# bmezaris/RetargetVid

Hardware: AMD Instinct MI355X
Metric: frames/sec end-to-end saliency+crop on 640x360 (higher is better)
Workload: dtype f32

## Files before the change

### retargetvid_amd/csrc/svc_net.hip

```cpp
#include <math.h>

#include <algorithm>

#include "svc_internal.h"
#include "svc_x3.h"

static inline int ceil_div(int a, int b) { return (a + b - 1) / b; }

__device__ __forceinline__ unsigned xcd_bx() {
    const unsigned b = blockIdx.x, n = gridDim.x;
    return (n & 7) ? b : (b & 7) * (n >> 3) + (b >> 3);
}

typedef float f32x2 __attribute__((ext_vector_type(2)));
__device__ __forceinline__ void fma4(float4 &a, const float4 x, const float4 w) {
    const f32x2 lo = __builtin_elementwise_fma((f32x2){x.x, x.y}, (f32x2){w.x, w.y}, (f32x2){a.x, a.y});
    const f32x2 hi = __builtin_elementwise_fma((f32x2){x.z, x.w}, (f32x2){w.z, w.w}, (f32x2){a.z, a.w});
    a = make_float4(lo.x, lo.y, hi.x, hi.y);
}


static thread_local char g_err[512] = "";
void svc_set_error(const char *fmt, ...) {
    va_list ap;
// ... 713 lines not shown
        }
#pragma unroll
        for (int ty = 0; ty < TY; ++ty) {
            const int ky = r - ty;
            if (ky < 0 || ky > 2) continue;
#pragma unroll
            for (int tx = 0; tx < TX; ++tx)
#pragma unroll
                for (int kx = 0; kx < 3; ++kx) {
                    const float4 x = row[tx + kx], ww = w[ky * 3 + kx];
                    acc[ty][tx].x = fmaf(x.x, ww.x, acc[ty][tx].x);
                    acc[ty][tx].y = fmaf(x.y, ww.y, acc[ty][tx].y);
                    acc[ty][tx].z = fmaf(x.z, ww.z, acc[ty][tx].z);
                    acc[ty][tx].w = fmaf(x.w, ww.w, acc[ty][tx].w);
                }
        }
    }
    const float4 b = *(const float4 *)(bias + c4 * 4);
    float *yf = Y + (size_t)f * H * W * C + c4 * 4;
#pragma unroll
    for (int ty = 0; ty < TY; ++ty)
#pragma unroll
        for (int tx = 0; tx < TX; ++tx) {
            if (oy0 + ty >= H || ox0 + tx >= W) continue;
            float4 v = acc[ty][tx];
            v.x = fminf(fmaxf(v.x + b.x, 0.f), 6.f);
            v.y = fminf(fmaxf(v.y + b.y, 0.f), 6.f);
            v.z = fminf(fmaxf(v.z + b.z, 0.f), 6.f);
            v.w = fminf(fmaxf(v.w + b.w, 0.f), 6.f);
            *(float4 *)(yf + ((size_t)(oy0 + ty) * W + ox0 + tx) * C) = v;
        }
}

__global__ __launch_bounds__(256) void k_subsample(const float *__restrict__ X, float *__restrict__ Y, int n, int H,
                                                   int W, int C) {
    const int C4 = C >> 2, OH = H >> 1, OW = W >> 1;
    size_t gid = (size_t)blockIdx.x * 256 + threadIdx.x;
    size_t total = (size_t)n * OH * OW * C4;
    if (gid >= total) return;
    int c4 = gid % C4;
    size_t pix = gid / C4;
    int ox = pix % OW, oy = (pix / OW) % OH, f = pix / ((size_t)OW * OH);
    *(float4 *)(Y + gid * 4) = *(const float4 *)(X + (((size_t)f * H + 2 * oy) * W + 2 * ox) * C + c4 * 4);
}

__global__ __launch_bounds__(256) void k_gauss_fill(const float *__restrict__ G, float *__restrict__ Y, int n,
                                                    int npos, int ldy, int c_off) {
    size_t gid = (size_t)blockIdx.x * 256 + threadIdx.x;
    size_t total = (size_t)n * npos * 16;
    if (gid >= total) return;
    int j = gid & 15;
    size_t fp = gid >> 4;
    int pos = fp % npos;
    Y[fp * ldy + c_off + j] = G[pos * 16 + j];
}

__global__ __launch_bounds__(256) void k_adapt(const float *__restrict__ X, const float *__restrict__ w,
                                               const float *__restrict__ b, float *__restrict__ Y, size_t npix,
                                               unsigned *__restrict__ fmax, int n, unsigned long long *__restrict__ census, int ncen) {
    size_t gid = (size_t)blockIdx.x * 256 + threadIdx.x;
    if (gid < (size_t)n) fmax[gid] = 0;
    if (census && gid < (size_t)ncen) {
        unsigned *pf = (unsigned *)(census + 4) + gid * 4;
#pragma unroll
        for (int j = 0; j < 3; ++j)
            if (pf[j]) { atomicAdd(census + j, (unsigned long long)pf[j]); pf[j] = 0; }
    }
    if (gid >= npix) return;
    const float4 *x = (const float4 *)(X + gid * 64);
    const float4 *w4 = (const float4 *)w;
    float s = 0.f;
#pragma unroll
    for (int i = 0; i < 16; ++i) {
        float4 a = x[i], c = w4[i];
        s = fmaf(a.x, c.x, s);
        s = fmaf(a.y, c.y, s);
        s = fmaf(a.z, c.z, s);
        s = fmaf(a.w, c.w, s);
    }
    Y[gid] = s + b[0];
}

__device__ __forceinline__ unsigned enc_f32(float v) {
    unsigned u = __float_as_uint(v);
    return (u & 0x80000000u) ? ~u : (u | 0x80000000u);
}
__device__ __forceinline__ float dec_f32(unsigned u) {
    return __uint_as_float((u & 0x80000000u) ? (u & 0x7FFFFFFFu) : ~u);
}

#ifdef SD_PACKED
#define SD_NO_PK
#else
#define SD_NO_PK SVC_NO_PK
#endif
__device__ __forceinline__ float sd_bilinear(float lx0, float lx1, float ly0, float ly1, float a00, float a01, float a10, float a11) {
#ifdef SD_PACKED
    return ly0 * (lx0 * a00 + lx1 * a01) + ly1 * (lx0 * a10 + lx1 * a11);
#else
    float p00, p01, p10, p11, r0, r1, q0, q1, v;
    asm volatile("v_mul_f32 %0, %1, %2" : "=v"(p00) : "v"(lx0), "v"(a00));
    asm volatile("v_mul_f32 %0, %1, %2" : "=v"(p01) : "v"(lx1), "v"(a01));
    asm volatile("v_mul_f32 %0, %1, %2" : "=v"(p10) : "v"(lx0), "v"(a10));
    asm volatile("v_mul_f32 %0, %1, %2" : "=v"(p11) : "v"(lx1), "v"(a11));
    asm volatile("v_add_f32 %0, %1, %2" : "=v"(r0) : "v"(p00), "v"(p01));
    asm volatile("v_add_f32 %0, %1, %2" : "=v"(r1) : "v"(p10), "v"(p11));
    asm volatile("v_mul_f32 %0, %1, %2" : "=v"(q0) : "v"(ly0), "v"(r0));
    asm volatile("v_mul_f32 %0, %1, %2" : "=v"(q1) : "v"(ly1), "v"(r1));
    asm volatile("v_add_f32 %0, %1, %2" : "=v"(v) : "v"(q0), "v"(q1));
    return v;
#endif
}

// ... 496 lines not shown
        SVC_CHECK_LAUNCH();
        return SVC_OK;
    }
    svc_set_error("no pointwise kernel for K = %d, N = %d%s", K, N, R ? " with a residual" : ups ? " with an up-sampled term" : "");
    return SVC_E_INVALID;
}

static int launch_pw(SvcHandle *h, hipStream_t s, const float *X, int ldx, const SvcLayer &L, const float *R, int ldr,
                     float *Y, int ldy, int M, int n) {
    return launch_pw_ex(h, s, X, ldx, L.w.dev, L.cin, L.cin, L.b.dev, L.relu6, L.cout, R, ldr, Y, ldy, M, n, nullptr);
}

static int launch_dw(SvcHandle *h, hipStream_t s, const float *X, const SvcLayer &L, float *Y, int n, int H, int W) {
    ProfScope ps(h, SVC_K_DW, s);
    const int C = L.cout, GX = (W + 3) / 4, GY = (H + 1) / 2;
    const size_t cells = (size_t)n * GY * GX * (C / 4);
    k_dw_tile<4, 2><<<blocks256(cells), 256, 0, s>>>(X, L.w.dev, L.b.dev, Y, n, H, W, C, make_fdiv(C / 4), make_fdiv(GX),
                                                     make_fdiv(GY), (uint32_t)cells);
    SVC_CHECK_LAUNCH();
    return SVC_OK;
}

#define IRB_ES 36
#ifndef IRB_XREG
#define IRB_XREG 1
#endif
#ifndef IRB_WAVES
#define IRB_WAVES 4
#endif
#ifndef IRB_STAMP
#define IRB_STAMP(i)
#endif

template <int NT, int PW, int NWV, bool MX = false>
__global__ __launch_bounds__(64 * NWV) __attribute__((amdgpu_waves_per_eu(2, 8))) void k_dwpw(const float *__restrict__ X, int H, int W, int C,
                                              const float *__restrict__ Wd, const float *__restrict__ bd,
                                              const float *__restrict__ Wp, const float *__restrict__ bp, int N,
                                              int Npad, const float *__restrict__ R, int ldr, float *__restrict__ Y,
                                              int ldy, int relu6, int tiles_x, int tiles_y, int lw_tiles) {
    constexpr int PH = 32 / PW;
    __shared__ float smem_dwpw[NWV * 32 * IRB_ES + NWV * 16 * 64];
    float (*Dw)[32 * IRB_ES] = (float (*)[32 * IRB_ES])smem_dwpw;
    float (*red)[16][64] = (float (*)[16][64])(smem_dwpw + NWV * 32 * IRB_ES);
    const int tid = threadIdx.x, lane = tid & 63, wave = tid >> 6, r = lane & 31, hh = lane >> 5;
    int bid = xcd_bx();
    const int tx = bid % tiles_x;
    bid /= tiles_x;
    const int ty = bid % tiles_y, f = bid / tiles_y;
    const int x0 = tx * PW, y0 = ty * PH, n0 = blockIdx.y * (NT * 32);
    const int c4 = lane & 7, p0 = (lane >> 3) * 4;
    const int py = p0 / PW, pxs = p0 % PW;
    const int oy = y0 + py, ox0 = x0 + pxs;
    const float *xf = X + (size_t)f * H * W * C;
    float *D = Dw[wave];
    f32x16 acc[NT];
#pragma unroll
    for (int t = 0; t < NT; ++t)
#pragma unroll
        for (int i = 0; i < 16; ++i) acc[t][i] = 0.f;
    const int nchunks = (C + 31) >> 5;
    constexpr bool PRE = false;
    const float *wrow[NT];
#pragma unroll
    for (int t = 0; t < NT; ++t)
        wrow[t] = lw_tiles ? Wp + ((size_t)min((int)blockIdx.y * NT + t, lw_tiles - 1) * 64 + lane) * 4
                           : Wp + (size_t)min(n0 + t * 32 + r, Npad - 1) * C + 4 * hh;
    const size_t wstep = lw_tiles ? (size_t)lw_tiles * 256 : 8;
    for (int ch = wave; ch < nchunks; ch += NWV) {
        const int kend = min(32, C - ch * 32);
        float4 Bw[PRE ? NT : 1][4];
        if (PRE) {
#pragma unroll
            for (int t = 0; t < NT; ++t)
#pragma unroll
                for (int q = 0; q < 4; ++q)
                    Bw[PRE ? t : 0][q] = *(const float4 *)(wrow[t] + wstep * (ch * 4 + min(q, (kend >> 3) - 1)));
        }
        const int c = ch * 32 + c4 * 4;
        const bool cok = c < C;
        const int cc = cok ? c : 0;
        float4 o[4];
#pragma unroll
        for (int j = 0; j < 4; ++j) o[j] = make_float4(0.f, 0.f, 0.f, 0.f);
        {
            float4 w[9];
#pragma unroll
            for (int t = 0; t < 9; ++t) w[t] = *(const float4 *)(Wd + (size_t)t * C + cc);
// ... 102 lines not shown
            }
        }
        __builtin_amdgcn_wave_barrier();
    }
    const int yy = y0 + r / PW, xx = x0 + r % PW;
    const bool live = yy < H && xx < W;
    const size_t pix = ((size_t)f * H + yy) * W + xx;
#pragma unroll
    for (int t = 0; t < NT; ++t) {
        if (t) __syncthreads();
#pragma unroll
        for (int i = 0; i < 16; ++i) red[wave][i][lane] = acc[t][i];
        __syncthreads();
        if (wave >= 4) continue;
        const int g = wave;
        const int col = n0 + t * 32 + 8 * g + 4 * hh;
        if (col >= N || !live) continue;
        float4 v = make_float4(red[0][4 * g][lane], red[0][4 * g + 1][lane], red[0][4 * g + 2][lane], red[0][4 * g + 3][lane]);
#pragma unroll
        for (int q = 1; q < NWV; ++q) {
            v.x += red[q][4 * g][lane]; v.y += red[q][4 * g + 1][lane];
            v.z += red[q][4 * g + 2][lane]; v.w += red[q][4 * g + 3][lane];
        }
        const float4 bv = *(const float4 *)(bp + col);
        v.x += bv.x; v.y += bv.y; v.z += bv.z; v.w += bv.w;
        if (R) {
            const float4 rv = *(const float4 *)(R + pix * ldr + col);
            v.x += rv.x; v.y += rv.y; v.z += rv.z; v.w += rv.w;
        }
        if (relu6) {
            v.x = fminf(fmaxf(v.x, 0.f), 6.f); v.y = fminf(fmaxf(v.y, 0.f), 6.f);
            v.z = fminf(fmaxf(v.z, 0.f), 6.f); v.w = fminf(fmaxf(v.w, 0.f), 6.f);
        }
        *(float4 *)(Y + pix * ldy + col) = v;
    }
}

template <int KS1, int NT2, bool MX = false>
__global__ __launch_bounds__(256) __attribute__((amdgpu_waves_per_eu(2, 8))) void k_pwpw(const float *__restrict__ X, int ldx, const float *__restrict__ W1,
                                              const float *__restrict__ b1, int Cm, const float *__restrict__ W2,
                                              const float *__restrict__ b2, float *__restrict__ Y, int ldy, int M, int lw) {
    constexpr int K1 = 8 * KS1;
    __shared__ float red_pp[4][16][64];
    const int tid = threadIdx.x, lane = tid & 63, wave = tid >> 6, r = lane & 31, hh = lane >> 5;
    const int m0 = xcd_bx() * 32;
    const float *xp = X + (size_t)min(m0 + r, M - 1) * ldx + 4 * hh;
    constexpr int Q1 = KS1 / 2;
    static_assert(KS1 % 2 == 0, "K1 must be a multiple of 16");
    float4 A1[MX ? 1 : KS1];
    X3 A13[MX ? Q1 : 1];
    if constexpr (MX) {
#pragma unroll
        for (int q = 0; q < Q1; ++q) A13[q] = x3_split(*(const float4 *)(xp + 16 * q), *(const float4 *)(xp + 16 * q + 8));
    } else {
#pragma unroll
        for (int p = 0; p < KS1; ++p) A1[MX ? 0 : p] = *(const float4 *)(xp + 8 * p);
    }
    f32x16 acc2[NT2];
#pragma unroll
    for (int t = 0; t < NT2; ++t)
#pragma unroll
        for (int i = 0; i < 16; ++i) acc2[t][i] = 0.f;
    const float *w2row[NT2];
#pragma unroll
    for (int t = 0; t < NT2; ++t) w2row[t] = lw ? W2 + ((size_t)t * 64 + lane) * 4 : W2 + (size_t)(t * 32 + r) * Cm + 4 * hh;
    const int nchunks = Cm >> 5;
    const size_t step2 = lw ? (size_t)NT2 * 256 : 8;
// ... 110 lines not shown
    ProfScope ps(h, SVC_K_PW, s);
    const bool k8 = L1.cin == 64 && L2.cout == 64, k20 = L1.cin == 160 && L2.cout == 128;
    if (!(k8 || k20) || (L1.cout % 32) != 0 || L2.cin != L1.cout || !L1.relu6 || L2.relu6) {
        svc_set_error("no k_pwpw instance for a %d -> %d -> %d skip branch", L1.cin, L1.cout, L2.cout);
        return SVC_E_INVALID;
    }
    const dim3 grid((unsigned)ceil_div(M, 32));
    const float *W1 = L1.w.dev, *W2 = L2.w.dev;
    int lw = 0;
    const bool mx = h->mx != 0;
    if (mx) {
        const uint4 *a = nullptr, *b = nullptr;
        int rc = x3_weights(h, s, L1.w.dev, L1.cin, L1.cin, L1.cout, X3_ROWS, &a);
        if (!rc) rc = x3_weights(h, s, L2.w.dev, L2.cin, L2.cin, L2.cout, X3_LANES, &b);
        if (rc) return rc;
        W1 = (const float *)a; W2 = (const float *)b;
        lw = 1;
    } else if (h->sk_lane) {
        int rc = lane_weights(h, s, L2.w.dev, L2.cin, L2.cin, L2.cout, &W2);
        if (rc) return rc;
        lw = 1;
    }
    const auto kfn = k8 ? (mx ? k_pwpw<8, 2, true> : k_pwpw<8, 2>) : (mx ? k_pwpw<20, 4, true> : k_pwpw<20, 4>);
    kfn<<<grid, 256, 0, s>>>(X, ldx, W1, L1.b.dev, L1.cout, W2, L2.b.dev, Y, ldy, M, lw);
    SVC_CHECK_LAUNCH();
    return SVC_OK;
}

#define DWPW_MAX_NT 5

static int dwpw_min_px(const SvcHandle *h) { return h->mx ? 100 : 400; }

static int launch_dwpw(SvcHandle *h, hipStream_t s, const float *X, const SvcLayer &Ld, const SvcLayer &Lp, const float *R,
                       int ldr, float *Y, int ldy, int n, int H, int W) {
    ProfScope ps(h, SVC_K_PW, s);
    const int C = Ld.cout, N = Lp.cout, Npad = (N + 31) / 32 * 32, tiles = Npad / 32;
    const int groups = ceil_div(tiles, DWPW_MAX_NT), nt = ceil_div(tiles, groups);
    const int pw = (W % 8 == 0 || W > 16) ? 8 : 16;
    const int tx = ceil_div(W, pw), ty = ceil_div(H, 32 / pw);
    dim3 grid((unsigned)(n * tx * ty), groups);
    const float *Wpl = Lp.w.dev;
    int lw_tiles = 0;
    const bool mx = h->mx && (C & 15) == 0;
    if (mx) {
        const uint4 *W3 = nullptr;
        int rc = x3_weights(h, s, Lp.w.dev, C, C, Npad, X3_LANES, &W3);
        if (rc) return rc;
        Wpl = (const float *)W3;
        lw_tiles = tiles;
    } else if (h->sk_lane && (C & 7) == 0) {
        int rc = lane_weights(h, s, Lp.w.dev, C, C, Npad, &Wpl);
        if (rc) return rc;
        lw_tiles = tiles;
    }
    decltype(&k_dwpw<2, 8, 4>) kfn = nullptr;
    if (pw == 8) {
        switch (nt) {
            case 2: kfn = mx ? k_dwpw<2, 8, 4, true> : k_dwpw<2, 8, 4>; break;
            case 3: kfn = mx ? k_dwpw<3, 8, 4, true> : k_dwpw<3, 8, 4>; break;
            case 4: kfn = mx ? k_dwpw<4, 8, 4, true> : k_dwpw<4, 8, 4>; break;
            case 5: kfn = mx ? k_dwpw<5, 8, 4, true> : k_dwpw<5, 8, 4>; break;
        }
    } else if (mx && nt == 4) kfn = k_dwpw<4, 16, 4, true>;
    else if (mx && nt == 5) kfn = k_dwpw<5, 16, 4, true>;
    if (!kfn) {
        svc_set_error("no k_dwpw instance for %d column tiles on a %d-wide level (%s pipe)", tiles, W, mx ? "split-bf16" : "fp32");
        return SVC_E_INVALID;
    }
    kfn<<<grid, 256, 0, s>>>(X, H, W, C, Ld.w.dev, Ld.b.dev, Wpl, Lp.b.dev, N, Npad, R, ldr, Y, ldy, Lp.relu6, tx, ty, lw_tiles);
    SVC_CHECK_LAUNCH();
    return SVC_OK;
}


template <int S, int TOH, int TOW>
struct IrbGeom {
    static constexpr int IH = (TOH - 1) * S + 3, IW = (TOW - 1) * S + 3, NPX = IH * IW, MT = (NPX + 31) / 32;
    static constexpr int NOUT = TOH * TOW;
    static size_t lds_floats(int Cin, int CoutP, bool expand, int Ce = 0, bool xreg = false, bool mx = false) {
        const size_t XS = Cin + 4;
        size_t n = (xreg ? 0 : (size_t)NPX * XS) + (expand ? (size_t)NPX * IRB_ES : 0) + (size_t)NOUT * IRB_ES;
        if (mx) n += 32 * (size_t)(((Cin + 15) / 16) * 6 + 1) * 4 + (CoutP == 64 ? (size_t)CoutP * 13 * 4 : (size_t)CoutP * IRB_ES) + 9 * 32;
        else n += (expand ? 32 * XS : 0) + (size_t)CoutP * IRB_ES + 9 * 32;
        n += 2 * (size_t)((Ce + 31) / 32 * 32);
        return n;
    }
};

template <int S, int TOH, int TOW, bool EXPAND, int CIN = 0, int CE = 0, int COUT = 0, bool MX = false>
#define IRB_MX3(S_, CIN_, COUT_, MX_) ((MX_) && (COUT_) == 64)
__global__ __launch_bounds__(256) __attribute__((amdgpu_waves_per_eu(IRB_MX3(S, CIN, COUT, MX) ? 3 : IRB_WAVES, 8))) void k_irb(const float *__restrict__ X, int H, int W, int Cin_,
                                             const float *__restrict__ We, const float *__restrict__ be, int Ce_,
                                             const float *__restrict__ Wd, const float *__restrict__ bd,
                                             const float *__restrict__ Wp, const float *__restrict__ bp, int Cout_,
                                             int CoutP_, const float *__restrict__ R, float *__restrict__ Y, int ldy_,
                                             int OH, int OW, int tiles_x, int tiles_y) {
    const int Cin = CIN > 0 ? CIN : Cin_, Ce = CE > 0 ? CE : Ce_, Cout = COUT > 0 ? COUT : Cout_;
    const int CoutP = COUT > 0 ? (COUT + 31) / 32 * 32 : CoutP_, ldy = COUT > 0 ? COUT : ldy_;
    using G = IrbGeom<S, TOH, TOW>;
    constexpr int IW = G::IW, NPX = G::NPX, MT = G::MT;
    constexpr int NOUT = G::NOUT, MP = NOUT / 32;
    extern __shared__ float sm_irb[];
    const int XS = Cin + 4;
    constexpr bool XREG = IRB_XREG && EXPAND && CIN > 0 && CIN <= 32 && (CIN % 8) == 0;
    static_assert(!MX || XREG, "the split-bf16 form exists for the fixed-shape expanding instances");
    constexpr bool MXP = MX && COUT == 64;
    constexpr int Q1 = MX ? (CIN + 15) / 16 : 1, RS1 = Q1 * 6 + 1;
    constexpr int QP = MXP ? (CE + 15) / 16 : 1;
    float *Xs = sm_irb;
    float *E = EXPAND ? Xs + (XREG ? 0 : NPX * XS) : Xs;
    float *D = E + NPX * IRB_ES;
    float *Wes = D + NOUT * IRB_ES;
    float *Wps = Wes + (MX ? 32 * RS1 * 4 : (EXPAND ? 32 * XS : 0));
    float *Wds = Wps + (MXP ? CoutP * 13 * 4 : CoutP * IRB_ES);
    uint4 *Wes3 = (uint4 *)Wes, *Wps3 = (uint4 *)Wps;
    float *Bes = Wds + 9 * 32;
    float *Bds = Bes + ((Ce + 31) / 32 * 32);
    const int tid = threadIdx.x, lane = tid & 63, wave = tid >> 6, r = lane & 31, hh = lane >> 5;
    int bid = xcd_bx();
    const int tx = bid % tiles_x;
    bid /= tiles_x;
    const int ty = bid % tiles_y, f = bid / tiles_y;
    const int oy0 = ty * TOH, ox0 = tx * TOW, iy0 = oy0 * S - 1, ix0 = ox0 * S - 1;
    const int c4n = Cin >> 2;
    const int nchunks = (Ce + 31) >> 5;
    const int we_n = MX ? (32 * Q1 * 6 + 255) >> 8 : EXPAND ? (32 * c4n + 255) >> 8 : 0;
    const bool wd_mine = tid < 72;
    const int wd_t = tid >> 3, wd_c4 = tid & 7;
    const int wp_n = MXP ? (CoutP * 12 + 255) >> 8 : (CoutP * 8 + 255) >> 8;
// ... 258 lines not shown
        if (!EXPAND) __syncthreads();
    }
    IRB_STAMP(7);
    if (KS > 1) {
        const int PS = CoutP + 4;
        float *Pp = sm_irb;
        __syncthreads();
        {
            const int pm = t0 % MP, nt = t0 / MP;
            float *pp = Pp + ((size_t)ks * NOUT + pm * 32 + r) * PS + nt * 32 + 4 * hh;
#pragma unroll
            for (int g = 0; g < 4; ++g)
                *(float4 *)(pp + 8 * g) = make_float4(acc[0][4 * g], acc[0][4 * g + 1], acc[0][4 * g + 2], acc[0][4 * g + 3]);
        }
        __syncthreads();
        const int c4o = CoutP >> 2;
        for (int idx = tid; idx < NOUT * c4o; idx += 256) {
            const int px = idx / c4o, col = (idx - px * c4o) * 4;
            const int oy = oy0 + px / TOW, ox = ox0 + px % TOW;
            if (col >= Cout || oy >= OH || ox >= OW) continue;
            float4 v = *(const float4 *)(Pp + (size_t)px * PS + col);
            for (int q = 1; q < KS; ++q) {
                const float4 t = *(const float4 *)(Pp + ((size_t)q * NOUT + px) * PS + col);
                v.x += t.x; v.y += t.y; v.z += t.z; v.w += t.w;
            }
            const float4 b = *(const float4 *)(bp + col);
            v.x += b.x; v.y += b.y; v.z += b.z; v.w += b.w;
            const size_t pix = ((size_t)f * OH + oy) * OW + ox;
            if (R) {
                const float4 rv = *(const float4 *)(R + pix * Cout + col);
                v.x += rv.x; v.y += rv.y; v.z += rv.z; v.w += rv.w;
            }
            *(float4 *)(Y + pix * ldy + col) = v;
        }
        return;
    }
#pragma unroll
    for (int j = 0; j < 2; ++j) {
        const int tile = t0 + 4 * j;
        if (tile >= ptiles) continue;
        const int pm = tile % MP, nt = tile / MP;
        const int px = pm * 32 + r;
        const int oy = oy0 + px / TOW, ox = ox0 + px % TOW;
        if (oy >= OH || ox >= OW) continue;
        const size_t pix = ((size_t)f * OH + oy) * OW + ox;
#pragma unroll
        for (int g = 0; g < 4; ++g) {
            const int col = nt * 32 + 8 * g + 4 * hh;
            if (col >= Cout) continue;
            const float4 bv = *(const float4 *)(bp + col);
            float4 v = make_float4(acc[j][4 * g] + bv.x, acc[j][4 * g + 1] + bv.y, acc[j][4 * g + 2] + bv.z, acc[j][4 * g + 3] + bv.w);
            if (R) {
                const float4 rv = *(const float4 *)(R + pix * Cout + col);
                v.x += rv.x; v.y += rv.y; v.z += rv.z; v.w += rv.w;
            }
            *(float4 *)(Y + pix * ldy + col) = v;
        }
    }
}

static int launch_irb(SvcHandle *h, hipStream_t s, const float *X, int n, int H, int W, int Cin, const SvcLayer *Le,
                      const SvcLayer &Ld, const SvcLayer &Lp, int stride, const float *R, float *Y) {
    ProfScope ps(h, SVC_K_PW, s);
    const int Ce = Ld.cout, Cout = Lp.cout, CoutP = (Cout + 31) / 32 * 32;
    const int OH = H / stride, OW = W / stride;
    const float *We_ = Le ? Le->w.dev : nullptr, *Wp_ = Lp.w.dev;
    auto mx_weights = [&]() -> int {
        const uint4 *a = nullptr, *b = nullptr;
        int rc = x3_weights(h, s, Le->w.dev, Cin, Cin, (Ce + 31) / 32 * 32, X3_ROWS, &a);
        We_ = (const float *)a;
        if (!rc && Cout == 64) {
            rc = x3_weights(h, s, Lp.w.dev, Ce, Ce, CoutP, X3_ROWS, &b);
            Wp_ = (const float *)b;
        }
        return rc;
    };
#define IRB_LAUNCH_MX(S_, TOH_, TOW_, CI_, CE_, CO_)                                                                 \
    do {                                                                                                             \
        if (h->mx) {                                                                                                 \
            int rc = mx_weights();                                                                                   \
            if (rc) return rc;                                                                                       \
            IRB_LAUNCH(S_, TOH_, TOW_, true, CI_, CE_, CO_, true);                                                   \
        } else IRB_LAUNCH(S_, TOH_, TOW_, true, CI_, CE_, CO_, false);                                               \
    } while (0)
#define IRB_LAUNCH(S_, TOH_, TOW_, EXP_, CI_, CE_, CO_, MX_)                                                         \
    do {                                                                                                             \
        const int tx = ceil_div(OW, TOW_), ty = ceil_div(OH, TOH_);                                                  \
        const size_t lds = IrbGeom<S_, TOH_, TOW_>::lds_floats(Cin, CoutP, EXP_, Ce, IRB_XREG && EXP_ && (CI_) > 0 && (CI_) <= 32 && ((CI_) % 8) == 0, MX_) * 4; \
        auto kfn = k_irb<S_, TOH_, TOW_, EXP_, CI_, CE_, CO_, MX_>;                                                  \
          \
          \
        if (h->lds_attr_done.insert((const void *)kfn).second)                                                       \
            SVC_HIP(hipFuncSetAttribute((const void *)kfn, hipFuncAttributeMaxDynamicSharedMemorySize, 120 * 1024)); \
        kfn<<<dim3((unsigned)(n * tx * ty)), 256, lds, s>>>(                                                          \
            X, H, W, Cin, EXP_ ? We_ : nullptr, EXP_ ? Le->b.dev : nullptr, Ce, Ld.w.dev, Ld.b.dev, Wp_,              \
            Lp.b.dev, Cout, CoutP, R, Y, Cout, OH, OW, tx, ty);                                                       \
    } while (0)
    if (!Le && Cin == 32 && Ce == 32 && Cout == 16) IRB_LAUNCH(1, 8, 8, false, 32, 32, 16, false);
    else if (!Le) {
        svc_set_error("no k_irb instance for a %d -> %d -> %d block without expansion", Cin, Ce, Cout);
        return SVC_E_INVALID;
    } else if (stride == 2 && Cin == 16 && Ce == 96 && Cout == 24) IRB_LAUNCH_MX(2, 4, 8, 16, 96, 24);
    else if (stride == 2 && Cin == 24 && Ce == 144 && Cout == 32) IRB_LAUNCH(2, 4, 8, true, 24, 144, 32, false);
    else if (stride == 1 && Cin == 24 && Ce == 144 && Cout == 24) IRB_LAUNCH_MX(1, 8, 8, 24, 144, 24);
    else if (stride == 1 && Cin == 32 && Ce == 192 && Cout == 32) IRB_LAUNCH_MX(1, 8, 8, 32, 192, 32);
    else if (stride == 1 && Cin == 32 && Ce == 192 && Cout == 64) IRB_LAUNCH_MX(1, 8, 8, 32, 192, 64);
    else {
        svc_set_error("no k_irb instance for a stride-%d %d -> %d -> %d block", stride, Cin, Ce, Cout);
        return SVC_E_INVALID;
    }
#undef IRB_LAUNCH_MX
#undef IRB_LAUNCH
    SVC_CHECK_LAUNCH();
    return SVC_OK;
}

#define RC(x) do { int rc_ = (x); if (rc_) return rc_; } while (0)

static int forward_chunk(SvcHandle *h, const uint8_t *frames, int n, uint8_t *maps, hipStream_t s, int thr = 0, unsigned *census_rows = nullptr,
                         unsigned *profile_rows = nullptr) {
    NetPlan *p = h->plan;
    const int NH = p->NH, NW = p->NW;
    int H = NH / 2, W = NW / 2;
    size_t li = 0;
    auto next = [&]() -> const SvcLayer & { return h->layers[li++]; };
    float *IN = p->buf(B_IN), *P[2] = {p->buf(B_P0), p->buf(B_P1)}, *E0 = p->buf(B_E0), *E1 = p->buf(B_E1);
    const int fr_lds = front_lds_bytes();
    const bool front = h->front && p->fr_ok;
    p->last_front = front;
    if (!front) {
        ProfScope ps(h, SVC_K_LANCZOS, s);
        dim3 grid(ceil_div(NH, LZ_ROWS), n);
        size_t lds = ((size_t)p->lz_tile_cap * p->w * 3 + 15) / 16 * 16 + ((size_t)p->lz_tile_cap * NW * 3 + 15) / 16 * 16 +
                     (size_t)NW * p->hks * 4 + 768 * 4;
        k_lanczos_norm<<<grid, 256, lds, s>>>(frames, IN, p->h, p->w, NH, NW, (const int *)p->hb.p, (const int *)p->hk.p,
                                             p->hks, (const int *)p->vb.p, (const int *)p->vk.p, p->vks,
                                             (const float *)p->lut.p, LZ_ROWS, p->lz_tile_cap);
        SVC_CHECK_LAUNCH();
    }
    const SvcLayer &Lstem = next();
    if (!front) {
        ProfScope ps(h, SVC_K_STEM, s);
        const int tx = ceil_div(W, STEM_TW), ty = ceil_div(H, STEM_TH);
        k_stem_mfma<<<dim3((unsigned)(n * tx * ty)), 256, 0, s>>>(IN, (const float *)h->stem_wt.p, Lstem.b.dev, P[0], NH, NW,
                                                                 H, W, tx, ty);
        SVC_CHECK_LAUNCH();
    }
    int cur = 0;
    static const int T[7] = {1, 6, 6, 6, 6, 6, 6}, Cc[7] = {16, 24, 32, 64, 96, 160, 320}, Nn[7] = {1, 2, 3, 4, 3, 3, 1},
                     Ss[7] = {1, 2, 2, 2, 1, 2, 1};
    int idx = 1, inp = 32;
    for (int st = 0; st < 7; ++st)
        for (int i = 0; i < Nn[st]; ++i, ++idx) {
            const int oup = Cc[st], stride = (i == 0) ? Ss[st] : 1, t = T[st];
            const bool res = (stride == 1 && inp == oup);
            const bool tap = (idx == 7 || idx == 14);
            const int dws = (stride == 2 && !tap) ? 2 : 1;
            const float *x = P[cur];
            int OH = H / dws, OW = W / dws;
            float *y = tap ? p->buf(idx == 7 ? B_F4X : B_F2X) : P[cur ^ 1];
            if (front && idx == 1) {
                ProfScope ps(h, SVC_K_STEM, s);
                const SvcLayer &Ld = next();
                const SvcLayer &Lp = next();
                FrontArgs A;
                A.frames = frames; A.h = p->h; A.w = p->w; A.NH = NH; A.NW = NW; A.OH = H; A.OW = W;
                A.tiles_x = ceil_div(W, FR_TW); A.tiles_y = ceil_div(H, FR_TH);
                A.hb = (const int *)p->hb.p; A.hk = (const int *)p->hk.p; A.vb = (const int *)p->vb.p; A.vk = (const int *)p->vk.p;
                A.hks = p->hks; A.vks = p->vks; A.lut = (const float *)p->lut.p;
                A.Wstem = (const float *)h->stem_wt.p; A.bstem = Lstem.b.dev;
                RC(lane_weights(h, s, (const float *)h->stem_wt.p, 32, 32, 32, &A.Wstem_l));
                RC(lane_weights(h, s, Lp.w.dev, 32, 32, 16, &A.Wp_l));
                A.Wd = Ld.w.dev; A.bd = Ld.b.dev; A.Wp = Lp.w.dev; A.bp = Lp.b.dev;
                A.Y = y; A.in_dbg = h->keep_input ? IN : nullptr;
                A.nr_cap = p->fr_nr; A.nc_cap = p->fr_nc;
                for (int i = 0; i < FR_MAXT; ++i) {
                    A.row_lo[i] = p->fr_row_lo[i]; A.row_n[i] = p->fr_row_n[i];
                    A.col_lo[i] = p->fr_col_lo[i]; A.col_n[i] = p->fr_col_n[i];
                }
                k_front<<<dim3((unsigned)(n * A.tiles_x * A.tiles_y)), 256, fr_lds, s>>>(A);
                SVC_CHECK_LAUNCH();
            } else if (idx <= 7) {
                const SvcLayer *Le = (t != 1) ? &next() : nullptr;
                const SvcLayer &Ld = next();
                const SvcLayer &Lp = next();
                RC(launch_irb(h, s, x, n, H, W, inp, Le, Ld, Lp, dws, res ? x : nullptr, y));
            } else {
                const float *dwin = x;
                if (t != 1) {
                    RC(launch_pw(h, s, x, inp, next(), nullptr, 0, E0, inp * t, n * H * W, n));
                    dwin = E0;
                }
                const SvcLayer &Ld = next();
                if (H * W >= dwpw_min_px(h)) {
                    const SvcLayer &Lp = next();
                    RC(launch_dwpw(h, s, dwin, Ld, Lp, res ? x : nullptr, oup, y, oup, n, H, W));
                } else {
                    RC(launch_dw(h, s, dwin, Ld, E1, n, H, W));
                    RC(launch_pw(h, s, E1, inp * t, next(), res ? x : nullptr, oup, y, oup, n * OH * OW, n));
                }
            }
            if (tap) {
                ProfScope ps(h, SVC_K_RESAMPLE, s);
                k_subsample<<<blocks256((size_t)n * (OH / 2) * (OW / 2) * (oup / 4)), 256, 0, s>>>(y, P[cur ^ 1], n, OH,
                                                                                                  OW, oup);
                SVC_CHECK_LAUNCH();
                OH /= 2; OW /= 2;
            }
            H = OH; W = OW;
            cur ^= 1;
            inp = oup;
        }
    const int H5 = H, W5 = W, H4 = 2 * H5, W4 = 2 * W5, H3 = 4 * H5, W3 = 4 * W5;
    float *CAT1 = p->buf(B_CAT1);
    RC(launch_pw(h, s, P[cur], 320, next(), nullptr, 0, CAT1, 1296, n * H5 * W5, n));
    float *CAT2 = p->buf(B_CAT2), *CAT3 = p->buf(B_CAT3);
    {
        const SvcLayer &Le2 = next();
        const SvcLayer &Lr2 = next();
        RC(launch_pwpw(h, s, p->buf(B_F2X), 160, Le2, Lr2, CAT2 + 256, 384, n * H4 * W4));
        const SvcLayer &Le4 = next();
        const SvcLayer &Lr4 = next();
        RC(launch_pwpw(h, s, p->buf(B_F4X), 64, Le4, Lr4, CAT3 + 128, 192, n * H3 * W3));
    }
    next();
    if (p->gauss_filled < n) {
        ProfScope ps(h, SVC_K_RESAMPLE, s);
        k_gauss_fill<<<blocks256((size_t)n * H5 * W5 * 16), 256, 0, s>>>((const float *)p->gauss.p, CAT1, n, H5 * W5,
                                                                         1296, 1280);
        SVC_CHECK_LAUNCH();
        p->gauss_filled = n;
    }
    if (H5 * W5 >= dwpw_min_px(h)) {
        const SvcLayer &Ld = next();
        RC(launch_dwpw(h, s, CAT1, Ld, next(), nullptr, 0, p->buf(B_PC), 256, n, H5, W5));
    } else {
        RC(launch_dw(h, s, CAT1, next(), p->buf(B_PCD), n, H5, W5));
        RC(launch_pw(h, s, p->buf(B_PCD), 1296, next(), nullptr, 0, p->buf(B_PC), 256, n * H5 * W5, n));
    }
    {
        const SvcLayer &Le = next();
        RC(launch_pw_ex(h, s, p->buf(B_PC), 256, Le.w.dev, 384, 256, nullptr, 0, 768, nullptr, 0, p->buf(B_T1), 768,
                        n * H5 * W5, n, nullptr));
        const UpsAdd ua{p->buf(B_T1), H5, W5, 768, make_fdiv(W4), make_fdiv(H4)};
        RC(launch_pw_ex(h, s, CAT2 + 256, 384, Le.w.dev + 256, 384, 128, Le.b.dev, Le.relu6, 768, nullptr, 0,
                        p->buf(B_U2E), 768, n * H4 * W4, n, &ua));
        const SvcLayer &Ld = next();
        RC(launch_dwpw(h, s, p->buf(B_U2E), Ld, next(), nullptr, 0, p->buf(B_U2), 128, n, H4, W4));
    }
    {
        const SvcLayer &Le = next();
        RC(launch_pw_ex(h, s, p->buf(B_U2), 128, Le.w.dev, 192, 128, nullptr, 0, 384, nullptr, 0, p->buf(B_T2), 384,
                        n * H4 * W4, n, nullptr));
        const UpsAdd ua{p->buf(B_T2), H4, W4, 384, make_fdiv(W3), make_fdiv(H3)};
        RC(launch_pw_ex(h, s, CAT3 + 128, 192, Le.w.dev + 128, 192, 64, Le.b.dev, Le.relu6, 384, nullptr, 0,
                        p->buf(B_P3E), 384, n * H3 * W3, n, &ua));
        const SvcLayer &Ld = next();
        RC(launch_dwpw(h, s, p->buf(B_P3E), Ld, next(), nullptr, 0, p->buf(B_DEC), 64, n, H3, W3));
    }
    const SvcLayer &La = next();
    {
        ProfScope ps(h, SVC_K_RESAMPLE, s);
        k_adapt<<<blocks256((size_t)n * H3 * W3), 256, 0, s>>>(p->buf(B_DEC), La.w.dev, La.b.dev, p->buf(B_LOGIT),
                                                              (size_t)n * H3 * W3, (unsigned *)p->fmax.p, n,
                                                              (unsigned long long *)h->census.p, h->chunk);
        SVC_CHECK_LAUNCH();
    }
    const SvcLayer &Ls = next();
    ProfScope ps_smooth(h, SVC_K_SMOOTH, s);
    {
        dim3 grid(ceil_div(p->h, SD_ROWS), n);
        const size_t lds = ((size_t)H3 * W3 + 64 * SD_KP + (size_t)p->sd_tile_cap * NW) * sizeof(float);
        k_smooth_down_mfma<<<grid, 256, lds, s>>>(p->buf(B_LOGIT), Ls.w.dev, p->buf(B_PRE), (unsigned *)p->fmax.p, H3, W3,
                                                  NH, NW, p->h, p->w, SD_ROWS, p->sd_tile_cap, make_fdiv(p->w));
        SVC_CHECK_LAUNCH();
    }
    if (profile_rows) {
        k_quantise_profile<<<dim3(ceil_div(p->h, BP_ROWS), n), 256, 0, s>>>(p->buf(B_PRE), (const unsigned *)p->fmax.p, maps, p->h, p->w,
                                                                            thr, (unsigned long long *)h->census.p, census_rows,
                                                                            profile_rows);
    } else {
        k_quantise<<<blocks256((size_t)n * p->h * p->w), 256, 0, s>>>(p->buf(B_PRE), (const unsigned *)p->fmax.p, maps, n,
                                                                     p->h * p->w, make_fdiv(p->h * p->w), thr,
                                                                     (unsigned long long *)h->census.p, census_rows);
    }
    SVC_CHECK_LAUNCH();
    if (thr > 0) h->census_maps += (unsigned long long)n;
    p->last_n = n;
    return SVC_OK;
}

static int saliency_impl(SvcHandle *h, const uint8_t *frames, int n, int height, int width, uint8_t *maps, int thr, void *stream,
                         uint32_t *census_rows = nullptr, uint32_t *profile_rows = nullptr);

extern "C" int svc_saliency_u8(SvcHandle *h, const uint8_t *frames, int n, int height, int width, uint8_t *maps,
                               void *stream) {
    return saliency_impl(h, frames, n, height, width, maps, 0, stream);
}

// ... 46 lines not shown
    if (n == 0) return SVC_OK;
    SVC_HIP(hipSetDevice(h->device));
    const int nb = std::min(n, h->chunk);
    RC(build_plan(h, height, width, nb));
    const size_t fin = (size_t)height * width * 3, fout = (size_t)height * width;
    hipStream_t s = (hipStream_t)stream;
    for (int i = 0; i < n; i += h->plan->nb) {
        int m = std::min(h->plan->nb, n - i);
        const uint8_t *fr = frames + i * fin;
        uint8_t *mp = maps + i * fout;
        RC(forward_chunk(h, fr, m, mp, s, thr, census_rows ? census_rows + (size_t)i * 4 : nullptr,
                         profile_rows ? profile_rows + (size_t)i * (height + width) : nullptr));
    }
    return SVC_OK;
}

extern "C" int svc_debug_tap(SvcHandle *h, int which, int frame, float *out_host, size_t cap_floats) {
    if (!h || !h->plan || !out_host) { svc_set_error("svc_debug_tap: no forward pass has run"); return SVC_E_INVALID; }
    NetPlan *p = h->plan;
    static const int map[7] = {B_IN, B_F4X, B_F2X, B_CAT1, B_PC, B_DEC, B_PRE};
    if (which < 0 || which > 6 || frame < 0 || frame >= p->last_n) { svc_set_error("svc_debug_tap: bad tap/frame"); return SVC_E_INVALID; }
    const int NH = p->NH, NW = p->NW;
    size_t count;
    switch (which) {
        case SVC_TAP_INPUT: count = (size_t)NH * NW * 3; break;
        case SVC_TAP_FEAT4X: count = (size_t)(NH / 8) * (NW / 8) * 64; break;
        case SVC_TAP_FEAT2X: count = (size_t)(NH / 16) * (NW / 16) * 160; break;
        case SVC_TAP_FEAT1X: count = (size_t)(NH / 32) * (NW / 32) * 1296; break;
        case SVC_TAP_POSTCNN: count = (size_t)(NH / 32) * (NW / 32) * 256; break;
        case SVC_TAP_DEC: count = (size_t)(NH / 8) * (NW / 8) * 64; break;
        default: count = (size_t)p->h * p->w; break;
    }
    if (count > cap_floats) { svc_set_error("svc_debug_tap: buffer too small (%zu needed)", count); return SVC_E_INVALID; }
    if (which == SVC_TAP_INPUT && p->last_front && !h->keep_input) {
        svc_set_error("svc_debug_tap: the fused front kernel keeps the network input on chip; create the handle with SVC_KEEP_INPUT=1 (or SVC_FRONT=0)");
        return SVC_E_INVALID;
    }
    SVC_HIP(hipSetDevice(h->device));
    SVC_HIP(hipDeviceSynchronize());
    SVC_HIP(hipMemcpy(out_host, p->buf(map[which]) + (size_t)frame * count, count * sizeof(float), hipMemcpyDeviceToHost));
    return (int)count;
}

extern "C" int svc_front_fused(const SvcHandle *h) { return h && h->plan && h->plan->last_front ? 1 : 0; }
extern "C" int svc_matrix_pipe(const SvcHandle *h) { return h ? h->mx : 0; }

extern "C" int svc_threshold_census(SvcHandle *h, unsigned long long *out, int reset) {
    if (!h || !out) { svc_set_error("svc_threshold_census: invalid argument"); return SVC_E_INVALID; }
    SVC_HIP(hipSetDevice(h->device));
    SVC_HIP(hipDeviceSynchronize());
    std::vector<unsigned char> host(h->census.bytes);
    SVC_HIP(hipMemcpy(host.data(), h->census.p, h->census.bytes, hipMemcpyDeviceToHost));
    const unsigned long long *tot = (const unsigned long long *)host.data();
    const unsigned *pf = (const unsigned *)(tot + 4);
    out[0] = h->census_maps;
    for (int j = 0; j < 3; ++j) {
        unsigned long long v = tot[j];
        for (int f = 0; f < h->chunk; ++f) v += pf[f * 4 + j];
        out[1 + j] = v;
    }
    if (reset) {
        SVC_HIP(hipMemset(h->census.p, 0, h->census.bytes));
        h->census_maps = 0;
    }
    return SVC_OK;
}
// ... 231 lines not shown
```

Before: 25560.

## Fuse subsample store and adaptation dot product into dwpw/irb epilogues

Removes the standalone k_subsample kernel by having the dwpw and irb epilogues write the even-pixel subsampled copy directly to the next ping-pong buffer. Removes k_adapt by computing the 64-channel adaptation dot product inside the final dwpw kernel through shared memory. Block 0 of that kernel also resets fmax and folds the census. The B_DEC tensor is no longer written unless keep_input is set. This saves two launches and a global round trip, at the cost of an extra template instance, a __syncthreads in the epilogue, and more restrictive shape checks.

```diff
diff --git a/retargetvid_amd/csrc/svc_net.hip b/retargetvid_amd/csrc/svc_net.hip
--- a/retargetvid_amd/csrc/svc_net.hip
+++ b/retargetvid_amd/csrc/svc_net.hip
@@ -769,18 +769,6 @@
         }
 }
 
-__global__ __launch_bounds__(256) void k_subsample(const float *__restrict__ X, float *__restrict__ Y, int n, int H,
-                                                   int W, int C) {
-    const int C4 = C >> 2, OH = H >> 1, OW = W >> 1;
-    size_t gid = (size_t)blockIdx.x * 256 + threadIdx.x;
-    size_t total = (size_t)n * OH * OW * C4;
-    if (gid >= total) return;
-    int c4 = gid % C4;
-    size_t pix = gid / C4;
-    int ox = pix % OW, oy = (pix / OW) % OH, f = pix / ((size_t)OW * OH);
-    *(float4 *)(Y + gid * 4) = *(const float4 *)(X + (((size_t)f * H + 2 * oy) * W + 2 * ox) * C + c4 * 4);
-}
-
 __global__ __launch_bounds__(256) void k_gauss_fill(const float *__restrict__ G, float *__restrict__ Y, int n,
                                                     int npos, int ldy, int c_off) {
     size_t gid = (size_t)blockIdx.x * 256 + threadIdx.x;
@@ -792,20 +780,8 @@
     Y[fp * ldy + c_off + j] = G[pos * 16 + j];
 }
 
-__global__ __launch_bounds__(256) void k_adapt(const float *__restrict__ X, const float *__restrict__ w,
-                                               const float *__restrict__ b, float *__restrict__ Y, size_t npix,
-                                               unsigned *__restrict__ fmax, int n, unsigned long long *__restrict__ census, int ncen) {
-    size_t gid = (size_t)blockIdx.x * 256 + threadIdx.x;
-    if (gid < (size_t)n) fmax[gid] = 0;
-    if (census && gid < (size_t)ncen) {
-        unsigned *pf = (unsigned *)(census + 4) + gid * 4;
-#pragma unroll
-        for (int j = 0; j < 3; ++j)
-            if (pf[j]) { atomicAdd(census + j, (unsigned long long)pf[j]); pf[j] = 0; }
-    }
-    if (gid >= npix) return;
-    const float4 *x = (const float4 *)(X + gid * 64);
-    const float4 *w4 = (const float4 *)w;
+__device__ __forceinline__ float adapt_dot(const float4 *x, const float4 *w4, const float *b) {
+#pragma clang fp contract(off) reassociate(off)
     float s = 0.f;
 #pragma unroll
     for (int i = 0; i < 16; ++i) {
@@ -815,7 +791,7 @@
         s = fmaf(a.z, c.z, s);
         s = fmaf(a.w, c.w, s);
     }
-    Y[gid] = s + b[0];
+    return s + b[0];
 }
 
 __device__ __forceinline__ unsigned enc_f32(float v) {
@@ -1378,12 +1354,23 @@
 #define IRB_STAMP(i)
 #endif
 
-template <int NT, int PW, int NWV, bool MX = false>
+struct AdaptOut {
+    const float *w, *b;
+    float *logit;
+    unsigned *fmax; int n;
+    unsigned long long *census; int ncen;
+};
+#define ADAPT_ES 68
+
+template <int NT, int PW, int NWV, bool MX = false, bool ADAPT = false>
 __global__ __launch_bounds__(64 * NWV) __attribute__((amdgpu_waves_per_eu(2, 8))) void k_dwpw(const float *__restrict__ X, int H, int W, int C,
                                               const float *__restrict__ Wd, const float *__restrict__ bd,
                                               const float *__restrict__ Wp, const float *__restrict__ bp, int N,
                                               int Npad, const float *__restrict__ R, int ldr, float *__restrict__ Y,
-                                              int ldy, int relu6, int tiles_x, int tiles_y, int lw_tiles) {
+                                              int ldy, int relu6, int tiles_x, int tiles_y, int lw_tiles,
+                                              float *__restrict__ Y2 = nullptr, const AdaptOut A = AdaptOut()) {
+    static_assert(!ADAPT || (NT == 2 && NWV == 4), "the adaptation epilogue needs every channel of the pixel in the workgroup");
+    static_assert(ADAPT_ES * 32 <= NWV * 32 * IRB_ES, "the 64-channel tile lies over the depthwise slabs");
     constexpr int PH = 32 / PW;
     __shared__ float smem_dwpw[NWV * 32 * IRB_ES + NWV * 16 * 64];
     float (*Dw)[32 * IRB_ES] = (float (*)[32 * IRB_ES])smem_dwpw;
@@ -1399,6 +1386,16 @@
     const int oy = y0 + py, ox0 = x0 + pxs;
     const float *xf = X + (size_t)f * H * W * C;
     float *D = Dw[wave];
+    if (ADAPT && blockIdx.x == 0) {
+        for (int i = tid; i < A.n; i += 64 * NWV) A.fmax[i] = 0;
+        if (A.census)
+            for (int i = tid; i < A.ncen; i += 64 * NWV) {
+                unsigned *pf = (unsigned *)(A.census + 4) + (size_t)i * 4;
+#pragma unroll
+                for (int j = 0; j < 3; ++j)
+                    if (pf[j]) { atomicAdd(A.census + j, (unsigned long long)pf[j]); pf[j] = 0; }
+            }
+    }
     f32x16 acc[NT];
 #pragma unroll
     for (int t = 0; t < NT; ++t)
@@ -1567,7 +1564,14 @@
             v.x = fminf(fmaxf(v.x, 0.f), 6.f); v.y = fminf(fmaxf(v.y, 0.f), 6.f);
             v.z = fminf(fmaxf(v.z, 0.f), 6.f); v.w = fminf(fmaxf(v.w, 0.f), 6.f);
         }
-        *(float4 *)(Y + pix * ldy + col) = v;
+        if (!ADAPT || Y) *(float4 *)(Y + pix * ldy + col) = v;
+        if (!ADAPT && Y2 && !((yy | xx) & 1) && (yy >> 1) < (H >> 1) && (xx >> 1) < (W >> 1))
+            *(float4 *)(Y2 + (((size_t)f * (H >> 1) + (yy >> 1)) * (W >> 1) + (xx >> 1)) * ldy + col) = v;
+        if (ADAPT) *(float4 *)(smem_dwpw + r * ADAPT_ES + col) = v;
+    }
+    if constexpr (ADAPT) {
+        __syncthreads();
+        if (tid < 32 && live) A.logit[pix] = adapt_dot((const float4 *)(smem_dwpw + tid * ADAPT_ES), (const float4 *)A.w, A.b);
     }
 }
 
@@ -1744,7 +1748,7 @@
 static int dwpw_min_px(const SvcHandle *h) { return h->mx ? 100 : 400; }
 
 static int launch_dwpw(SvcHandle *h, hipStream_t s, const float *X, const SvcLayer &Ld, const SvcLayer &Lp, const float *R,
-                       int ldr, float *Y, int ldy, int n, int H, int W) {
+                       int ldr, float *Y, int ldy, int n, int H, int W, float *Y2 = nullptr, const AdaptOut *adapt = nullptr) {
     ProfScope ps(h, SVC_K_PW, s);
     const int C = Ld.cout, N = Lp.cout, Npad = (N + 31) / 32 * 32, tiles = Npad / 32;
     const int groups = ceil_div(tiles, DWPW_MAX_NT), nt = ceil_div(tiles, groups);
@@ -1765,8 +1769,17 @@
         if (rc) return rc;
         lw_tiles = tiles;
     }
+    if (Y2 && (((H | W) & 1) || adapt)) {
+        svc_set_error("k_dwpw: no sub-sampled store on a level of odd size (%d x %d) or next to the adaptation", H, W);
+        return SVC_E_INVALID;
+    }
+    if (adapt && (N != 64 || nt != 2 || pw != 8 || R)) {
+        svc_set_error("k_dwpw: the adaptation epilogue needs a 64-channel layer without residual in 8 x 4 patches (%d channels, %d-wide level)", N, W);
+        return SVC_E_INVALID;
+    }
     decltype(&k_dwpw<2, 8, 4>) kfn = nullptr;
-    if (pw == 8) {
+    if (adapt) kfn = mx ? k_dwpw<2, 8, 4, true, true> : k_dwpw<2, 8, 4, false, true>;
+    else if (pw == 8) {
         switch (nt) {
             case 2: kfn = mx ? k_dwpw<2, 8, 4, true> : k_dwpw<2, 8, 4>; break;
             case 3: kfn = mx ? k_dwpw<3, 8, 4, true> : k_dwpw<3, 8, 4>; break;
@@ -1779,7 +1792,8 @@
         svc_set_error("no k_dwpw instance for %d column tiles on a %d-wide level (%s pipe)", tiles, W, mx ? "split-bf16" : "fp32");
         return SVC_E_INVALID;
     }
-    kfn<<<grid, 256, 0, s>>>(X, H, W, C, Ld.w.dev, Ld.b.dev, Wpl, Lp.b.dev, N, Npad, R, ldr, Y, ldy, Lp.relu6, tx, ty, lw_tiles);
+    kfn<<<grid, 256, 0, s>>>(X, H, W, C, Ld.w.dev, Ld.b.dev, Wpl, Lp.b.dev, N, Npad, R, ldr, Y, ldy, Lp.relu6, tx, ty, lw_tiles, Y2,
+                             adapt ? *adapt : AdaptOut());
     SVC_CHECK_LAUNCH();
     return SVC_OK;
 }
@@ -1806,7 +1820,7 @@
                                              const float *__restrict__ Wd, const float *__restrict__ bd,
                                              const float *__restrict__ Wp, const float *__restrict__ bp, int Cout_,
                                              int CoutP_, const float *__restrict__ R, float *__restrict__ Y, int ldy_,
-                                             int OH, int OW, int tiles_x, int tiles_y) {
+                                             int OH, int OW, int tiles_x, int tiles_y, float *__restrict__ Y2 = nullptr) {
     const int Cin = CIN > 0 ? CIN : Cin_, Ce = CE > 0 ? CE : Ce_, Cout = COUT > 0 ? COUT : Cout_;
     const int CoutP = COUT > 0 ? (COUT + 31) / 32 * 32 : CoutP_, ldy = COUT > 0 ? COUT : ldy_;
     using G = IrbGeom<S, TOH, TOW>;
@@ -2131,6 +2145,8 @@
                 v.x += rv.x; v.y += rv.y; v.z += rv.z; v.w += rv.w;
             }
             *(float4 *)(Y + pix * ldy + col) = v;
+            if (Y2 && !((oy | ox) & 1) && (oy >> 1) < (OH >> 1) && (ox >> 1) < (OW >> 1))
+                *(float4 *)(Y2 + (((size_t)f * (OH >> 1) + (oy >> 1)) * (OW >> 1) + (ox >> 1)) * ldy + col) = v;
         }
         return;
     }
@@ -2154,15 +2170,21 @@
                 v.x += rv.x; v.y += rv.y; v.z += rv.z; v.w += rv.w;
             }
             *(float4 *)(Y + pix * ldy + col) = v;
+            if (Y2 && !((oy | ox) & 1) && (oy >> 1) < (OH >> 1) && (ox >> 1) < (OW >> 1))
+                *(float4 *)(Y2 + (((size_t)f * (OH >> 1) + (oy >> 1)) * (OW >> 1) + (ox >> 1)) * ldy + col) = v;
         }
     }
 }
 
 static int launch_irb(SvcHandle *h, hipStream_t s, const float *X, int n, int H, int W, int Cin, const SvcLayer *Le,
-                      const SvcLayer &Ld, const SvcLayer &Lp, int stride, const float *R, float *Y) {
+                      const SvcLayer &Ld, const SvcLayer &Lp, int stride, const float *R, float *Y, float *Y2 = nullptr) {
     ProfScope ps(h, SVC_K_PW, s);
     const int Ce = Ld.cout, Cout = Lp.cout, CoutP = (Cout + 31) / 32 * 32;
     const int OH = H / stride, OW = W / stride;
+    if (Y2 && ((OH | OW) & 1)) {
+        svc_set_error("k_irb: no sub-sampled store on a level of odd size (%d x %d)", OH, OW);
+        return SVC_E_INVALID;
+    }
     const float *We_ = Le ? Le->w.dev : nullptr, *Wp_ = Lp.w.dev;
     auto mx_weights = [&]() -> int {
         const uint4 *a = nullptr, *b = nullptr;
@@ -2193,7 +2215,7 @@
             SVC_HIP(hipFuncSetAttribute((const void *)kfn, hipFuncAttributeMaxDynamicSharedMemorySize, 120 * 1024)); \
         kfn<<<dim3((unsigned)(n * tx * ty)), 256, lds, s>>>(                                                          \
             X, H, W, Cin, EXP_ ? We_ : nullptr, EXP_ ? Le->b.dev : nullptr, Ce, Ld.w.dev, Ld.b.dev, Wp_,              \
-            Lp.b.dev, Cout, CoutP, R, Y, Cout, OH, OW, tx, ty);                                                       \
+            Lp.b.dev, Cout, CoutP, R, Y, Cout, OH, OW, tx, ty, Y2);                                                   \
     } while (0)
     if (!Le && Cin == 32 && Ce == 32 && Cout == 16) IRB_LAUNCH(1, 8, 8, false, 32, 32, 16, false);
     else if (!Le) {
@@ -2258,6 +2280,7 @@
             const float *x = P[cur];
             int OH = H / dws, OW = W / dws;
             float *y = tap ? p->buf(idx == 7 ? B_F4X : B_F2X) : P[cur ^ 1];
+            float *y2 = tap ? P[cur ^ 1] : nullptr;
             if (front && idx == 1) {
                 ProfScope ps(h, SVC_K_STEM, s);
                 const SvcLayer &Ld = next();
@@ -2283,7 +2306,7 @@
                 const SvcLayer *Le = (t != 1) ? &next() : nullptr;
                 const SvcLayer &Ld = next();
                 const SvcLayer &Lp = next();
-                RC(launch_irb(h, s, x, n, H, W, inp, Le, Ld, Lp, dws, res ? x : nullptr, y));
+                RC(launch_irb(h, s, x, n, H, W, inp, Le, Ld, Lp, dws, res ? x : nullptr, y, y2));
             } else {
                 const float *dwin = x;
                 if (t != 1) {
@@ -2293,19 +2316,16 @@
                 const SvcLayer &Ld = next();
                 if (H * W >= dwpw_min_px(h)) {
                     const SvcLayer &Lp = next();
-                    RC(launch_dwpw(h, s, dwin, Ld, Lp, res ? x : nullptr, oup, y, oup, n, H, W));
+                    RC(launch_dwpw(h, s, dwin, Ld, Lp, res ? x : nullptr, oup, y, oup, n, H, W, y2));
+                } else if (tap) {
+                    svc_set_error("block %d on a %d x %d level: only the fused depthwise + project kernel has the sub-sampled store", idx, H, W);
+                    return SVC_E_INVALID;
                 } else {
                     RC(launch_dw(h, s, dwin, Ld, E1, n, H, W));
                     RC(launch_pw(h, s, E1, inp * t, next(), res ? x : nullptr, oup, y, oup, n * OH * OW, n));
                 }
             }
-            if (tap) {
-                ProfScope ps(h, SVC_K_RESAMPLE, s);
-                k_subsample<<<blocks256((size_t)n * (OH / 2) * (OW / 2) * (oup / 4)), 256, 0, s>>>(y, P[cur ^ 1], n, OH,
-                                                                                                  OW, oup);
-                SVC_CHECK_LAUNCH();
-                OH /= 2; OW /= 2;
-            }
+            if (tap) { OH /= 2; OW /= 2; }
             H = OH; W = OW;
             cur ^= 1;
             inp = oup;
@@ -2355,15 +2375,10 @@
         RC(launch_pw_ex(h, s, CAT3 + 128, 192, Le.w.dev + 128, 192, 64, Le.b.dev, Le.relu6, 384, nullptr, 0,
                         p->buf(B_P3E), 384, n * H3 * W3, n, &ua));
         const SvcLayer &Ld = next();
-        RC(launch_dwpw(h, s, p->buf(B_P3E), Ld, next(), nullptr, 0, p->buf(B_DEC), 64, n, H3, W3));
-    }
-    const SvcLayer &La = next();
-    {
-        ProfScope ps(h, SVC_K_RESAMPLE, s);
-        k_adapt<<<blocks256((size_t)n * H3 * W3), 256, 0, s>>>(p->buf(B_DEC), La.w.dev, La.b.dev, p->buf(B_LOGIT),
-                                                              (size_t)n * H3 * W3, (unsigned *)p->fmax.p, n,
-                                                              (unsigned long long *)h->census.p, h->chunk);
-        SVC_CHECK_LAUNCH();
+        const SvcLayer &Lp = next();
+        const SvcLayer &La = next();
+        const AdaptOut ao{La.w.dev, La.b.dev, p->buf(B_LOGIT), (unsigned *)p->fmax.p, n, (unsigned long long *)h->census.p, h->chunk};
+        RC(launch_dwpw(h, s, p->buf(B_P3E), Ld, Lp, nullptr, 0, h->keep_input ? p->buf(B_DEC) : nullptr, 64, n, H3, W3, nullptr, &ao));
     }
     const SvcLayer &Ls = next();
     ProfScope ps_smooth(h, SVC_K_SMOOTH, s);
@@ -2476,6 +2491,10 @@
         default: count = (size_t)p->h * p->w; break;
     }
     if (count > cap_floats) { svc_set_error("svc_debug_tap: buffer too small (%zu needed)", count); return SVC_E_INVALID; }
+    if (which == SVC_TAP_DEC && !h->keep_input) {
+        svc_set_error("svc_debug_tap: the last decoder block's output goes straight into the adaptation layer; create the handle with SVC_KEEP_INPUT=1");
+        return SVC_E_INVALID;
+    }
     if (which == SVC_TAP_INPUT && p->last_front && !h->keep_input) {
         svc_set_error("svc_debug_tap: the fused front kernel keeps the network input on chip; create the handle with SVC_KEEP_INPUT=1 (or SVC_FRONT=0)");
         return SVC_E_INVALID;
```

Result: no change. 25660, median of 3 (+0.4%).
